# Antibas/eaQHM-analysis-and-synthesis-in-Python

Measured on AMD Instinct MI355X. Metric: analysis_frames_per_sec, higher is better.
Workload: dtype f64; 1 GPU; synth16k_60s_female_maxAdpt5; samples=960000, fs=16000, ls_frames_per_adaptation=63936, adaptations_executed=5, Kmax=59, track_bytes=906240000, parallelism=instants sharded x1 by LS cost; boundary records all-gathered per adaptation

## Files before the change

eaqhm-analysis-and-synthesis-in-python_amd/csrc/eaqhm_ls_tile.hip:

```cpp
#include <type_traits>
#include "eaqhm_ls_common.h"
#include "eaqhm_ls_chol.h"
#include "eaqhm_ls_a0.h"
#include "eaqhm_ls_tilemap.h"
#include "eaqhm_ls_twunits.h"
#include "eaqhm_ls_gather.h"
#include "eaqhm_ls_tilelds.h"

namespace eaqhm {
bool ls_a0tile_fits(const LsArgs& A);
int launch_ls_a0tile(eaqhm_ctx* ctx, LsArgs A);

#define DIAG_OWNER(jb, nt) ((int)TL_DIAG[nt][jb])
#define TL_THREADS 512
#define TL_WAVES 8
#define TL_CW 8
static_assert(TLL_TILE == TL_TILE && TLL_DG_TILE == DG_TILE, "eaqhm_ls_tilelds.h and eaqhm_ls_chol.h disagree");

__device__ inline void fetch_next_header(const LsArgs& A, TlHead* hd, int C, int nbuf, int lane) {
  int* cls = uni(A.cls);
  int item = 0;
  if (lane == 0) item = atomicAdd(cls + 8 + C, 1);
  item = uni(item);
  int f = -1;
  if (item < uni(cls[C])) f = uni(cls[16 + (size_t)C * uni(A.n_frames) + item]);
  if (f >= 0) {
    const int* tab = (lane == 0) ? A.ncol : (lane == 1) ? A.frame_c : (lane == 2) ? A.frame_wl : A.frame_inst;
    if (lane < 4) (&hd->n)[lane] = tab[f];
    const int Kmax = uni(A.Kmax);
    if (lane < TL_NSLOT && lane < Kmax) hd->cols[nbuf][lane] = A.cols[(size_t)f * Kmax + lane];
  }
  if (lane == 0) { hd->f = f; hd->buf = nbuf; hd->cls = C; }
}

__device__ inline void tw_step(d4 (&g)[9], double aR, double aI, double bR, double bI, double nk) {
  const double sA = aR + aI, dB = bI - bR;
  const double naR = nk * aR, naI = nk * aI, nsA = nk * sA;
  const double nbR = nk * bR, nbI = nk * bI, ndB = nk * dB;
  g[0] = __builtin_amdgcn_mfma_f64_16x16x4f64(aR, bR, g[0], 0, 0, 0);
  g[1] = __builtin_amdgcn_mfma_f64_16x16x4f64(aI, bI, g[1], 0, 0, 0);
  g[2] = __builtin_amdgcn_mfma_f64_16x16x4f64(sA, dB, g[2], 0, 0, 0);
  g[3] = __builtin_amdgcn_mfma_f64_16x16x4f64(naR, bR, g[3], 0, 0, 0);
  g[4] = __builtin_amdgcn_mfma_f64_16x16x4f64(naI, bI, g[4], 0, 0, 0);
  g[5] = __builtin_amdgcn_mfma_f64_16x16x4f64(nsA, dB, g[5], 0, 0, 0);
  g[6] = __builtin_amdgcn_mfma_f64_16x16x4f64(naR, nbR, g[6], 0, 0, 0);
  g[7] = __builtin_amdgcn_mfma_f64_16x16x4f64(naI, nbI, g[7], 0, 0, 0);
  g[8] = __builtin_amdgcn_mfma_f64_16x16x4f64(nsA, ndB, g[8], 0, 0, 0);
}

__device__ inline void twu_pair_k3(d4 (&g0)[3], d4 (&g1)[3], d4 (&g2)[3], double aR, double aI, double bR, double bI, double nk) {
  const double sA = aR + aI, dB = bI - bR;
  const double naR = nk * aR, naI = nk * aI, nsA = nk * sA;
  const double nbR = nk * bR, nbI = nk * bI, ndB = nk * dB;
  g0[0] = __builtin_amdgcn_mfma_f64_16x16x4f64(aR, bR, g0[0], 0, 0, 0);
  g0[1] = __builtin_amdgcn_mfma_f64_16x16x4f64(aI, bI, g0[1], 0, 0, 0);
  g0[2] = __builtin_amdgcn_mfma_f64_16x16x4f64(sA, dB, g0[2], 0, 0, 0);
  g1[0] = __builtin_amdgcn_mfma_f64_16x16x4f64(naR, bR, g1[0], 0, 0, 0);
  g1[1] = __builtin_amdgcn_mfma_f64_16x16x4f64(naI, bI, g1[1], 0, 0, 0);
  g1[2] = __builtin_amdgcn_mfma_f64_16x16x4f64(nsA, dB, g1[2], 0, 0, 0);
  g2[0] = __builtin_amdgcn_mfma_f64_16x16x4f64(naR, nbR, g2[0], 0, 0, 0);
  g2[1] = __builtin_amdgcn_mfma_f64_16x16x4f64(naI, nbI, g2[1], 0, 0, 0);
  g2[2] = __builtin_amdgcn_mfma_f64_16x16x4f64(nsA, ndB, g2[2], 0, 0, 0);
}
__device__ inline void twu_pair_2acc(d4 (&g0)[2], d4 (&g1)[2], d4 (&g2)[2], double aR, double aI, double bR, double bI, double nk,
                                     bool k4) {
  const double naR = nk * aR, naI = nk * aI, nbR = nk * bR, nbI = nk * bI;
  g0[0] = __builtin_amdgcn_mfma_f64_16x16x4f64(aR, bR, g0[0], 0, 0, 0);
  g1[0] = __builtin_amdgcn_mfma_f64_16x16x4f64(naR, bR, g1[0], 0, 0, 0);
  g2[0] = __builtin_amdgcn_mfma_f64_16x16x4f64(naR, nbR, g2[0], 0, 0, 0);
  g0[1] = __builtin_amdgcn_mfma_f64_16x16x4f64(aR, bI, g0[1], 0, 0, 0);
  g1[1] = __builtin_amdgcn_mfma_f64_16x16x4f64(naR, bI, g1[1], 0, 0, 0);
  g2[1] = __builtin_amdgcn_mfma_f64_16x16x4f64(naR, nbI, g2[1], 0, 0, 0);
  g0[0] = __builtin_amdgcn_mfma_f64_16x16x4f64(aI, bI, g0[0], 0, 0, 0);
  g1[0] = __builtin_amdgcn_mfma_f64_16x16x4f64(naI, bI, g1[0], 0, 0, 0);
  g2[0] = __builtin_amdgcn_mfma_f64_16x16x4f64(naI, nbI, g2[0], 0, 0, 0);
  if (k4) {
    const double maI = -aI, mnaI = -naI;
    g0[1] = __builtin_amdgcn_mfma_f64_16x16x4f64(maI, bR, g0[1], 0, 0, 0);
    g1[1] = __builtin_amdgcn_mfma_f64_16x16x4f64(mnaI, bR, g1[1], 0, 0, 0);
    g2[1] = __builtin_amdgcn_mfma_f64_16x16x4f64(mnaI, nbR, g2[1], 0, 0, 0);
  }
}

__device__ inline void twu_edge_k4(d4 (&g0)[2], d4 (&g1)[2], double aR, double aI, double bR, double bI, double nk) {
  const double nbR = nk * bR, nbI = nk * bI, maI = -aI;
  g0[0] = __builtin_amdgcn_mfma_f64_16x16x4f64(aR, bR, g0[0], 0, 0, 0);
  g1[0] = __builtin_amdgcn_mfma_f64_16x16x4f64(aR, nbR, g1[0], 0, 0, 0);
  g0[1] = __builtin_amdgcn_mfma_f64_16x16x4f64(aR, bI, g0[1], 0, 0, 0);
  g1[1] = __builtin_amdgcn_mfma_f64_16x16x4f64(aR, nbI, g1[1], 0, 0, 0);
  g0[0] = __builtin_amdgcn_mfma_f64_16x16x4f64(aI, bI, g0[0], 0, 0, 0);
  g1[0] = __builtin_amdgcn_mfma_f64_16x16x4f64(aI, nbI, g1[0], 0, 0, 0);
  g0[1] = __builtin_amdgcn_mfma_f64_16x16x4f64(maI, bR, g0[1], 0, 0, 0);
  g1[1] = __builtin_amdgcn_mfma_f64_16x16x4f64(maI, nbR, g1[1], 0, 0, 0);
}

template <int NS, int TW, int UA = 0, int UB = 0, int TB = 0>
__device__ __attribute__((noinline)) void tile_frame(const LsArgs& A, int TS_, int ldx_max_, double* lds, int f_) {
  constexpr int C = NS == 12 ? 5 : NS == 10 ? 4 : NS == 9 ? 3 : NS == 7 ? 2 : NS == 6 ? 1 : 0;
  static_assert(NS == 12 || NS == 10 || NS == 9 || NS == 7 || NS == 6 || NS == 5, "a register budget per class");
  constexpr bool NEXT_HEAD = NS != 10, REC_ROW = NS == 9;
  const bool pre = uni(f_) < 0;
  const int TS = uni(TS_), ldx_max = uni(ldx_max_);
  const int tid = threadIdx.x, nt_thr = TL_THREADS;
  const int lane = tid & 63;
  const int wave = __builtin_amdgcn_readfirstlane(tid >> 6);
  double* U = uni(lds);
  TlHead* hd = (TlHead*)(U + tl_head_offset());
  const int f = pre ? uni(hd->f) : uni(f_);
  double* Xre = U;
  double* Xim = Xre + (size_t)TS * ldx_max;
  const size_t usize_g = (size_t)2 * TS * ldx_max;
  double* ci = U + usize_g;
  unsigned long long* masks = (unsigned long long*)(ci + (size_t)CI_STRIDE * 52);
  double* PanR = U;
  double* PanI = PanR + TL_NTMAX * TL_TILE;
  double* WtR = PanI + TL_NTMAX * TL_TILE;
  double* WtI = WtR + TL_NTMAX * TL_TILE;
  double* LdR = WtI + TL_NTMAX * TL_TILE;
  double* LdI = LdR + TL_TILE;
  double* Dc = LdI + TL_TILE;
  double* Zc = Dc + DG_TILE;
  double* zv = Zc + DG_TILE;
  double* xv = zv + 2 * 16 * TL_NTMAX;
  double* xs = xv + 32 + TL_HEAD_DOUBLES;
  double* sh = xs + 4 * uni(A.Kcmax);
  double* win = sh + 16;
  double* sig = win + 64 * CI_NCH;
  double* dorig = sig + 64 * CI_NCH;

  const int Npad = ((uni(A.Nmax) + 63) >> 6) << 6;
  double* Qs = uni(A.scratch) + (size_t)blockIdx.x * (size_t)uni((int)A.scratch_stride);
  double* Rs = Qs + (size_t)Npad * uni(A.nmax);
  const bool seeds = uni(hd->seeds) != 0;
  const double w1 = uni(2.0 * M_PI / A.fs);
  const int PE = TS / 2;
  const double* sA = uni(A.s);
  const int lcol = lane & 15, lq = lane >> 4;
  unsigned long long* dbg = uni(A.debug);
  unsigned long long t_prev = 0;

  {
    const int n = pre ? uni(hd->n) : uni(A.ncol[f]);
    const int Kc = 2 * n + 1, Ms = 2 * Kc + 1;
    const int nt = (Ms + 15) >> 4;
    const int c = pre ? uni(hd->c) : uni(A.frame_c[f]), wl = pre ? uni(hd->wl) : uni(A.frame_wl[f]);
    const int inst = pre ? uni(hd->inst) : uni(A.frame_inst[f]);
    const int N = 2 * wl + 1, mid = wl;
    const int T = (Kc + 16) >> 4;
    constexpr int UN = UA + UB;
    constexpr int GA = UA / 3, GB = UB / 3;
    constexpr bool G3 = TW > 0 || UN > 0;
    static_assert(TW == 0 || UN == 0, "whole pairs or units");
    static_assert(UN == 0 || (UA == TWU_UA && UB == TWU_UB), "slot layout of eaqhm_ls_twunits.h");
    static_assert(TB >= 0 && TB < TWU_NTB, "unit table");
    constexpr bool PK = UN > 0 && TWU_PACKED[TB];
    constexpr int EC = 16 * (TWU_TT[TB] - 1);
    const int nb = G3 ? T : nt;
    const int ldx = (nb << 4) + ((nb & 1) ? 0 : 16);
    const int npair = T * (T + 1) / 2;
    const int is = 2 * Kc - 16 * (nt - 1);
    const double f0 = uni(A.f0_stale);
    const int* mycols = pre ? (const int*)hd->cols[uni(hd->buf)] : uni(A.cols) + (size_t)f * uni(A.Kmax);
    const int npairs = mid + 1;

    if (dbg && tid == 0) {
      t_prev = __builtin_amdgcn_s_memtime();
      if (hd->t_last && !uni((int)A.debug_diag)) atomicAdd(dbg + 11, t_prev - hd->t_last);
    }
    double sv[2];
#pragma unroll
    for (int r = 0; r < 2; ++r) {
      const int t = tid + r * nt_thr;
      sv[r] = (t < N) ? sA[(size_t)(c - wl) + t] : 0.0;
    }
    for (int q = tid; q < TS * ldx; q += nt_thr) { Xre[q] = 0.0; Xim[q] = 0.0; }
#pragma unroll
    for (int r = 0; r < 2; ++r) {
      const int t = tid + r * nt_thr;
      if (t < N) { win[t] = window_value(false, t, N); sig[t] = sv[r]; }
    }
    int* gappy = (int*)(masks + (size_t)52 * CI_NCH);
    prepare_slots<CI_STRIDE, TL_WAVES>(A, Qs, Rs, Npad, ci, masks, gappy, mycols, n, N, mid, c, wl, seeds, lane, wave, CI_NCH,
                                       REC_ROW ? hd->fmc : nullptr);
    LS_STAMP(0);

    constexpr int NM3 = (NS <= 7) ? NS : 0;
    d4 accR[NS], accI[NS], acc3[NM3 ? NM3 : 1];
    int tP[NS], tQ[NS];
    bool live[NS];
#pragma unroll
    for (int sl = 0; sl < NS; ++sl) {
      accR[sl] = (d4){0, 0, 0, 0};
      accI[sl] = (d4){0, 0, 0, 0};
      if (sl < NM3) acc3[sl] = (d4){0, 0, 0, 0};
      const int code = TL_MAP[nt][wave][sl];
      live[sl] = code != 0xFF;
      const int P = live[sl] ? (code >> 4) : 0, Q = live[sl] ? (code & 15) : 0;
      tP[sl] = __builtin_amdgcn_readfirstlane(P);
      tQ[sl] = __builtin_amdgcn_readfirstlane(Q);
    }

    constexpr int TWA = TW ? TW : 1;
    const bool split = TW > 0 && NS == 5 && T == 4;
    d4 g[TWA][9];
    int gI[TWA], gJ[TWA], gx[TWA];
    bool glive[TWA];
#pragma unroll
    for (int sl = 0; sl < TWA; ++sl) {
      const int x = (split && sl == 1) ? 8 + (wave >> 1) : wave + 8 * sl;
      glive[sl] = TW && x < npair && !(split && sl == 1 && wave >= 4);
      gx[sl] = __builtin_amdgcn_readfirstlane(x);
      int I = 0, J = 0;
      if (glive[sl]) tile_of(x, I, J);
      gI[sl] = __builtin_amdgcn_readfirstlane(I);
      gJ[sl] = __builtin_amdgcn_readfirstlane(J);
#pragma unroll
      for (int p = 0; p < 9; ++p) g[sl][p] = (d4){0, 0, 0, 0};
    }

    constexpr int UAA = UA > 3 ? UA : 3, UBA = UB > 3 ? UB : 3;
    d4 ga[UAA][3], gb[UBA][2];
    int ucode[UN ? UN : 1];
    if constexpr (UN > 0) {
#pragma unroll
      for (int sl = 0; sl < UN; ++sl) ucode[sl] = __builtin_amdgcn_readfirstlane((int)TWU_MAPS[TB][wave][sl]);
#pragma unroll
      for (int sl = 0; sl < UA; ++sl)
#pragma unroll
        for (int p = 0; p < 3; ++p) ga[sl][p] = (d4){0, 0, 0, 0};
#pragma unroll
      for (int sl = 0; sl < UB; ++sl) gb[sl][0] = gb[sl][1] = (d4){0, 0, 0, 0};
    }

    for (int d0 = 0; d0 < npairs; d0 += PE) {
#pragma clang loop unroll(disable)
      for (int idx = tid; idx < 16 * n; idx += nt_thr) {
        const int el = idx & 15, j = idx >> 4, d = d0 + el;
        const bool act = d <= mid;
        const int u = mid - d - 1, v = mid + d;
        double su = 0, cu = 1, sv, cv;
        double pur = 0, pui = 0, nur = 0, nui = 0, pvr, pvi, nvr, nvi;
        {
          double* cj = ci + j * CI_STRIDE;
          const double* fb = ((const double**)cj)[2];
          const double* ab = ((const double**)cj)[3];
          const int dc = act ? d : mid;
          const double fu1 = fb[mid - dc], fv = fb[mid + dc];
          const double au = ab[(mid - dc - 1 >= 0) ? (mid - dc - 1) : 0], au1 = ab[mid - dc];
          const double av = ab[mid + dc], av1 = ab[(mid + dc + 1 < N) ? (mid + dc + 1) : (N - 1)];
          const double xu = act ? fu1 : 0.0, xv = (act && d >= 1) ? fv : 0.0;
          const double qv = cj[0] + scan16(xv), qu = -(cj[1] + scan16(xu));
          if (el == 15) { cj[0] = qv; cj[1] = -qu; }
          if (!act) continue;
          const double ainv = cj[17], pr = cj[18], pi = cj[19];
          sincos_cw(qu * w1, &su, &cu);
          sincos_cw(qv * w1, &sv, &cv);
          const double eps = 10e-5;
          if (u >= 0) {
            const double ru = (eps + au) * ainv, rv1 = (eps + av1) * ainv;
            pur = ru * cu;                    pui = ru * su;
            nur = rv1 * (cv * pr - sv * pi);  nui = rv1 * (cv * pi + sv * pr);
          }
          const double rv = (eps + av) * ainv, ru1 = (eps + au1) * ainv;
          pvr = rv * cv;                      pvi = rv * sv;
          nvr = ru1 * (cu * pr - su * pi);    nvi = ru1 * (cu * pi + su * pr);
        }
        double* xr = Xre + (2 * el) * ldx;
        double* xi = Xim + (2 * el) * ldx;
        const int cpos = XCOL(n + 1 + j, el), cneg = XCOL(j, el);
        const int spos = XCOL(Kc + n + 1 + j, el), sneg = XCOL(Kc + j, el);
        const double wv = win[v], nv = (double)(v - mid);
        if (u >= 0) {
          const double wu = win[u], nu = (double)(u - mid);
          pur *= wu; pui *= wu; nur *= wu; nui *= wu;
          xr[cpos] = pur;      xi[cpos] = pui;      xr[cneg] = nur;      xi[cneg] = nui;
          if (!G3) { xr[spos] = nu * pur; xi[spos] = nu * pui; xr[sneg] = nu * nur; xi[sneg] = nu * nui; }
          if (PK && n + 1 + j >= EC) { xr[XCOL(n + 9 + j, el)] = nu * pur; xi[XCOL(n + 9 + j, el)] = nu * pui; }
        }
        pvr *= wv; pvi *= wv; nvr *= wv; nvi *= wv;
        xr += ldx; xi += ldx;
        xr[cpos] = pvr;      xi[cpos] = pvi;      xr[cneg] = nvr;      xi[cneg] = nvi;
        if (!G3) { xr[spos] = nv * pvr; xi[spos] = nv * pvi; xr[sneg] = nv * nvr; xi[sneg] = nv * nvi; }
        if (PK && n + 1 + j >= EC) { xr[XCOL(n + 9 + j, el)] = nv * pvr; xi[XCOL(n + 9 + j, el)] = nv * pvi; }
      }
      if ((tid & 15) == 0 && (tid >> 4) < TS) {
        const int row = tid >> 4;
        const int d = d0 + (row >> 1);
        const int t = (row & 1) ? (mid + d) : (mid - d - 1);
        const bool ok = (d <= mid) && (t >= 0);
        const double w = ok ? win[t] : 0.0;
        const double sval = ok ? sig[t] : 0.0;
        const double nn = (double)(t - mid);
        const int el = row >> 1;
        double* xr = Xre + row * ldx;
        double* xi = Xim + row * ldx;
        xr[XCOL(n, el)] = w;               xi[XCOL(n, el)] = 0.0;
        if (!G3) {
          xr[XCOL(Kc + n, el)] = w * nn;   xi[XCOL(Kc + n, el)] = 0.0;
        }
        const int scol = G3 ? Kc : 2 * Kc;
        xr[XCOL(scol, el)] = w * sval;     xi[XCOL(scol, el)] = 0.0;
        if (PK) { xr[XCOL(Kc + 8, el)] = w * sval * nn;  xi[XCOL(Kc + 8, el)] = 0.0; }
      }
      if (d0 + PE > mid) {
        for (int q = tid; q < TS * 16 * nb; q += nt_thr) {
          const int row = q / (16 * nb), col = q - row * (16 * nb);
          const int d = d0 + (row >> 1);
          const int t = (row & 1) ? (mid + d) : (mid - d - 1);
          if (d > mid || t < 0) { Xre[row * ldx + col] = 0.0; Xim[row * ldx + col] = 0.0; }
        }
      }
      LS_STAMP(12);
      __syncthreads();
      LS_STAMP(1);
      const int pcs = (npairs - d0 < PE) ? (npairs - d0) : PE;
      const int ksl = (pcs + 1) >> 1;
      if constexpr (UN > 0) {
        const int plane = TS * ldx_max;
        const int kn = (ksl < 8) ? ksl : 8;
#pragma unroll
        for (int gi = 0; gi < GA + GB; ++gi) {
          const int s0 = (gi < GA) ? 3 * gi : UA + 3 * (gi - GA);
          const int code = ucode[s0];
          if (code == 0xFFFF) continue;
          const int ca = 16 * ((code >> 8) & 15), cb = 16 * ((code >> 4) & 15);
          const bool k4 = (code & 3) == 1;
          int rb = lq * ldx;
          const int sw0 = lcol + (lq >> 1);
          int nk = (lq & 1) ? d0 + (lq >> 1) : -d0 - (lq >> 1) - 1;
          asm volatile("" : "+v"(rb), "+v"(nk));
          if (PK && gi >= GA) {
            if (code & 0x1000) {
              const int q = (gi >= GA) ? 3 * (gi - GA) : 0;
#pragma clang loop unroll(disable)
              for (int ks = 0; ks < kn; ++ks) {
                const int sw = (sw0 + 2 * ks) & 15;
                const double aR = Xre[rb + ca + sw], aI = Xre[rb + ca + sw + plane];
                const double bR = Xre[rb + cb + sw], bI = Xre[rb + cb + sw + plane];
                rb += 4 * ldx;
                twu_edge_k4(gb[q], gb[q + 1], aR, aI, bR, bI, (double)nk);
                nk += (lq & 1) ? 2 : -2;
              }
              continue;
            }
          }
#pragma clang loop unroll(disable)
          for (int ks = 0; ks < kn; ++ks) {
            const int sw = (sw0 + 2 * ks) & 15;
            const double aR = Xre[rb + ca + sw], aI = Xre[rb + ca + sw + plane];
            const double bR = Xre[rb + cb + sw], bI = Xre[rb + cb + sw + plane];
            rb += 4 * ldx;
            if (gi < GA) {
              const int q = (gi < GA) ? 3 * gi : 0;
              twu_pair_k3(ga[q], ga[q + 1], ga[q + 2], aR, aI, bR, bI, (double)nk);
            } else {
              const int q = (gi >= GA) ? 3 * (gi - GA) : 0;
              twu_pair_2acc(gb[q], gb[q + 1], gb[q + 2], aR, aI, bR, bI, (double)nk, k4);
            }
            nk += (lq & 1) ? 2 : -2;
          }
        }
#pragma unroll
        for (int sl = 0; sl < UN; ++sl) {
          if ((sl < UA) ? (sl < 3 * GA) : (sl - UA < 3 * GB)) continue;
          const int code = ucode[sl];
          if (code == 0xFFFF) continue;
          const int ca = 16 * ((code >> 8) & 15), cb = 16 * ((code >> 4) & 15), up = (code >> 2) & 3;
          const bool k4 = (code & 3) == 1;
          int rb = lq * ldx;
          const int sw0 = lcol + (lq >> 1);
          int nk = (lq & 1) ? d0 + (lq >> 1) : -d0 - (lq >> 1) - 1;
          asm volatile("" : "+v"(rb), "+v"(nk));
          auto run = [&](auto pc) {
            constexpr int P = decltype(pc)::value;
#pragma clang loop unroll(disable)
            for (int ks = 0; ks < kn; ++ks) {
              const int sw = (sw0 + 2 * ks) & 15;
              double aR = Xre[rb + ca + sw], aI = Xre[rb + ca + sw + plane];
              double bR = Xre[rb + cb + sw], bI = Xre[rb + cb + sw + plane];
              rb += 4 * ldx;
              if constexpr (P == 1 || P == 2) { aR *= (double)nk; aI *= (double)nk; }
              if constexpr (P >= 2) { bR *= (double)nk; bI *= (double)nk; }
              nk += (lq & 1) ? 2 : -2;
              if (sl < UA) {
                d4 (&g)[3] = ga[sl < UA ? sl : 0];
                g[0] = __builtin_amdgcn_mfma_f64_16x16x4f64(aR, bR, g[0], 0, 0, 0);
                g[1] = __builtin_amdgcn_mfma_f64_16x16x4f64(aI, bI, g[1], 0, 0, 0);
                g[2] = __builtin_amdgcn_mfma_f64_16x16x4f64(aR + aI, bI - bR, g[2], 0, 0, 0);
              } else {
                d4 (&g)[2] = gb[sl >= UA ? sl - UA : 0];
                g[0] = __builtin_amdgcn_mfma_f64_16x16x4f64(aR, bR, g[0], 0, 0, 0);
                g[1] = __builtin_amdgcn_mfma_f64_16x16x4f64(aR, bI, g[1], 0, 0, 0);
                g[0] = __builtin_amdgcn_mfma_f64_16x16x4f64(aI, bI, g[0], 0, 0, 0);
                if (k4) g[1] = __builtin_amdgcn_mfma_f64_16x16x4f64(-aI, bR, g[1], 0, 0, 0);
              }
            }
          };
          if (up == 0) run(std::integral_constant<int, 0>{});
          else if (PK && (code & 0x1000)) run(std::integral_constant<int, PK ? 3 : 1>{});
          else if (up == 1) run(std::integral_constant<int, 1>{});
          else run(std::integral_constant<int, 2>{});
        }
      } else if constexpr (TW > 0) {
#pragma unroll
        for (int sl = 0; sl < TW; ++sl) {
          if (!glive[sl]) continue;
          const int ca = 16 * gI[sl], cb = 16 * gJ[sl];
          int rb = lq * ldx;
          const int sw0 = lcol + (lq >> 1);
          int nk = (lq & 1) ? d0 + (lq >> 1) : -d0 - (lq >> 1) - 1;
          asm volatile("" : "+v"(rb), "+v"(nk));
          const int plane = TS * ldx_max;
          int kn = (ksl < 8) ? ksl : 8;
          int ks = 0;
          if (split && sl == 1) {
            if (wave & 1) { ks = 4; rb += 16 * ldx; nk += (lq & 1) ? 8 : -8; }
            else kn = (kn < 4) ? kn : 4;
          }
#pragma clang loop unroll(disable)
          for (; ks < kn; ++ks) {
            const int sw = (sw0 + 2 * ks) & 15;
            const double aR = Xre[rb + ca + sw], aI = Xre[rb + ca + sw + plane];
            const double bR = Xre[rb + cb + sw], bI = Xre[rb + cb + sw + plane];
            rb += 4 * ldx;
            tw_step(g[sl], aR, aI, bR, bI, (double)nk);
            nk += (lq & 1) ? 2 : -2;
          }
        }
      } else {
#pragma unroll
        for (int sl = 0; sl < NS; ++sl) {
          if (!live[sl]) continue;
          const int ca = 16 * tP[sl], cb = 16 * tQ[sl];
          int rb = lq * ldx;
          const int sw0 = lcol + (lq >> 1);
          asm volatile("" : "+v"(rb));
          const int plane = TS * ldx_max;
          if (ksl < 8) {
#pragma clang loop unroll(disable)
            for (int ks = 0; ks < ksl; ++ks) {
              const int sw = (sw0 + 2 * ks) & 15;
              const double aR = Xre[rb + ca + sw], aI = Xre[rb + ca + sw + plane];
              const double bR = Xre[rb + cb + sw], bI = Xre[rb + cb + sw + plane];
              rb += 4 * ldx;
              if (sl < NM3) {
                accR[sl] = __builtin_amdgcn_mfma_f64_16x16x4f64(aR, bR, accR[sl], 0, 0, 0);
                acc3[sl < NM3 ? sl : 0] = __builtin_amdgcn_mfma_f64_16x16x4f64(aI, bI, acc3[sl < NM3 ? sl : 0], 0, 0, 0);
                accI[sl] = __builtin_amdgcn_mfma_f64_16x16x4f64(aR + aI, bI - bR, accI[sl], 0, 0, 0);
              } else {
                accR[sl] = __builtin_amdgcn_mfma_f64_16x16x4f64(aR, bR, accR[sl], 0, 0, 0);
                accI[sl] = __builtin_amdgcn_mfma_f64_16x16x4f64(aR, bI, accI[sl], 0, 0, 0);
                accR[sl] = __builtin_amdgcn_mfma_f64_16x16x4f64(aI, bI, accR[sl], 0, 0, 0);
                accI[sl] = __builtin_amdgcn_mfma_f64_16x16x4f64(-aI, bR, accI[sl], 0, 0, 0);
              }
            }
            continue;
          }
          double aR, aI, bR, bI;
          {
            const int sw = sw0 & 15;
            aR = Xre[rb + ca + sw]; aI = Xre[rb + ca + sw + plane]; bR = Xre[rb + cb + sw]; bI = Xre[rb + cb + sw + plane];
          }
#pragma unroll
          for (int ks = 0; ks < 8; ++ks) {
            double naR = 0, naI = 0, nbR = 0, nbI = 0;
            if (ks < 7) {
              rb += 4 * ldx;
              const int sw = (sw0 + 2 * (ks + 1)) & 15;
              naR = Xre[rb + ca + sw]; naI = Xre[rb + ca + sw + plane]; nbR = Xre[rb + cb + sw]; nbI = Xre[rb + cb + sw + plane];
            }
            __builtin_amdgcn_sched_barrier(0);
            if (sl < NM3) {
              accR[sl] = __builtin_amdgcn_mfma_f64_16x16x4f64(aR, bR, accR[sl], 0, 0, 0);
              acc3[sl < NM3 ? sl : 0] = __builtin_amdgcn_mfma_f64_16x16x4f64(aI, bI, acc3[sl < NM3 ? sl : 0], 0, 0, 0);
              accI[sl] = __builtin_amdgcn_mfma_f64_16x16x4f64(aR + aI, bI - bR, accI[sl], 0, 0, 0);
            } else {
              accR[sl] = __builtin_amdgcn_mfma_f64_16x16x4f64(aR, bR, accR[sl], 0, 0, 0);
              accI[sl] = __builtin_amdgcn_mfma_f64_16x16x4f64(aR, bI, accI[sl], 0, 0, 0);
              accR[sl] = __builtin_amdgcn_mfma_f64_16x16x4f64(aI, bI, accR[sl], 0, 0, 0);
              accI[sl] = __builtin_amdgcn_mfma_f64_16x16x4f64(-aI, bR, accI[sl], 0, 0, 0);
            }
            aR = naR; aI = naI; bR = nbR; bI = nbI;
          }
        }
      }
      __syncthreads();
      LS_STAMP(2);
    }
    if constexpr (TW == 0 && NM3 > 0) {
#pragma unroll
      for (int sl = 0; sl < NM3; ++sl) {
        const d4 p1 = accR[sl], p2 = acc3[sl];
        accR[sl] = p1 + p2;
        accI[sl] = accI[sl] + (p1 - p2);
      }
    }
    if constexpr (G3) {
      double* Gs = Qs;
      int4* gtab = (int4*)U;
      if (tid < 16 * nt) {
        const GatherEntry e = gather_entry(tid, Kc, npair, T, PK);
        gtab[2 * tid] = make_int4(e.lo, e.hi, e.trow, e.tcol);
        if constexpr (PK) gtab[2 * tid + 1] = make_int4(e.mask, e.val, 0, 0);
      }
      if (tid == TL_THREADS - 1) *(double2*)((char*)Gs + GI_ZCELL) = make_double2(0.0, 0.0);
      if constexpr (UN > 0) {
#pragma unroll
        for (int sl = 0; sl < UN; ++sl) {
          const int code = ucode[sl];
          if (code == 0xFFFF) continue;
          const int I = (code >> 8) & 15, J = (code >> 4) & 15, up = (code >> 2) & 3;
          d4 re, im;
          if (sl < UA) {
            const d4 p1 = ga[sl < UA ? sl : 0][0], p2 = ga[sl < UA ? sl : 0][1];
            re = p1 + p2; im = ga[sl < UA ? sl : 0][2] + (p1 - p2);
          } else {
            re = gb[sl >= UA ? sl - UA : 0][0]; im = gb[sl >= UA ? sl - UA : 0][1];
          }
          double* gt = Gs + (size_t)(up * npair + I * (I + 1) / 2 + J) * 512;
#pragma unroll
          for (int r = 0; r < 4; ++r) {
            const int o = 2 * (16 * (lq + 4 * r) + lcol);
            gt[o] = re[r]; gt[o + 1] = im[r];
          }
        }
      } else
#pragma unroll
      for (int sl = 0; sl < TWA; ++sl) {
        if (!glive[sl]) continue;
        const int x = gx[sl];
        const bool second = split && sl == 1 && (wave & 1);
#pragma unroll
        for (int p = 0; p < 3; ++p) {
          const d4 p1 = g[sl][3 * p], p2 = g[sl][3 * p + 1];
          const d4 re = p1 + p2, im = g[sl][3 * p + 2] + (p1 - p2);
          double* gt = Gs + (size_t)(second ? 3 * npair + 3 * (x - 8) + p : p * npair + x) * 512;
#pragma unroll
          for (int r = 0; r < 4; ++r) {
            const int o = 2 * (16 * (lq + 4 * r) + lcol);
            gt[o] = re[r]; gt[o + 1] = im[r];
          }
        }
      }
      __syncthreads();
      if (split) {
        double2 c1[3], c2[3];
#pragma unroll
        for (int k = 0; k < 3; ++k) {
          const int q = tid + k * TL_THREADS, t = q >> 8, e = 2 * (q & 255);
          c1[k] = *(const double2*)(Gs + (size_t)((t % 3) * npair + 8 + t / 3) * 512 + e);
          c2[k] = *(const double2*)(Gs + (size_t)(3 * npair + t) * 512 + e);
        }
#pragma unroll
        for (int k = 0; k < 3; ++k) {
          const int q = tid + k * TL_THREADS, t = q >> 8, e = 2 * (q & 255);
          *(double2*)(Gs + (size_t)((t % 3) * npair + 8 + t / 3) * 512 + e) = make_double2(c1[k].x + c2[k].x, c1[k].y + c2[k].y);
        }
        __syncthreads();
      }
      if constexpr (UN > 0) {
        constexpr int TT = TWU_TT[TB], HN = (PK ? 3 * (TT - 1) + 1 : 3 * TT) * 136, HF = HN / TL_THREADS, HT = HF + (HN % TL_THREADS ? 1 : 0);
        double ha[HT], hb[HT];
        int hoa[HT], hob[HT];
#pragma unroll
        for (int k = 0; k < HT; ++k) {
          const int q = tid + k * TL_THREADS, qc = (q < HN) ? q : 0;
          const int t = qc / 136, e = qc - 136 * t, r = e / 17, c = e - 17 * r;
          const int i = (c < 16 - r) ? r : 15 - r, j = (c < 16 - r) ? r + c : c - 1;
          const int TD = PK ? TT - 1 : TT, pl = (t < 3 * TD) ? t / TD : 0, I = (t < 3 * TD) ? t - pl * TD : TT - 1;
          const int tile = (pl * npair + I * (I + 1) / 2 + I) * 512;
          hoa[k] = tile + 2 * (16 * i + j) + 1; hob[k] = tile + 2 * (16 * j + i) + 1;
          ha[k] = Gs[hoa[k]]; hb[k] = Gs[hob[k]];
        }
#pragma unroll
        for (int k = 0; k < HT; ++k) {
          if (k < HF || tid + k * TL_THREADS < HN) {
            Gs[hoa[k]] = ha[k] - hb[k];
            Gs[hob[k]] = hb[k] - ha[k];
          }
        }
        __syncthreads();
      }
      typedef const __attribute__((address_space(1))) char* gather_base_t;
      gather_base_t Gb = (gather_base_t)(const char*)Gs;
      unsigned gup[NS];
#pragma unroll
      for (int sl = 0; sl < NS; ++sl) {
        const int cx = live[sl] ? 16 * tQ[sl] + lcol : 16 * nt - 1;
        const int4* rt = gtab + 2 * (16 * tP[sl] + lq);
        int4 c0 = gtab[2 * cx], c1 = make_int4(0, 0, 0, 0), r0[4], r1[4];
        if constexpr (PK) c1 = gtab[2 * cx + 1];
#pragma unroll
        for (int r = 0; r < 4; ++r) {
          r0[r] = rt[8 * r];
          if constexpr (PK) r1[r] = rt[8 * r + 1];
        }
        asm volatile("" : "+v"(c0.x), "+v"(c0.y), "+v"(c0.w));
        if constexpr (PK) asm volatile("" : "+v"(c1.x), "+v"(c1.y));
#pragma unroll
        for (int r = 0; r < 4; ++r) {
          asm volatile("" : "+v"(r0[r].x), "+v"(r0[r].y), "+v"(r0[r].z));
          if constexpr (PK) asm volatile("" : "+v"(r1[r].x), "+v"(r1[r].y));
        }
        unsigned ups = 0;
#pragma unroll
        for (int r = 0; r < 4; ++r) {
          const int dt = r0[r].z - c0.w;
          unsigned off = (unsigned)((dt < 0 ? r0[r].y : r0[r].x) + (dt < 0 ? c0.x : c0.y));
          if constexpr (PK) off += (unsigned)((dt < 0 ? c1.x : r1[r].x) & (dt < 0 ? r1[r].y : c1.y));
          off = off < (unsigned)GI_ZCELL ? off : (unsigned)GI_ZCELL;
          ups = (ups >> 1) | ((unsigned)dt & 0x80000000u);
          typedef double gather_d2 __attribute__((ext_vector_type(2)));
          const gather_d2 v = *(const __attribute__((address_space(1))) gather_d2*)(Gb + off);
          accR[sl][r] = v.x; accI[sl][r] = v.y;
        }
        gup[sl] = ups;
      }
      __builtin_amdgcn_sched_barrier(0);
#pragma unroll
      for (int sl = 0; sl < NS; ++sl) {
#pragma unroll
        for (int r = 0; r < 4; ++r) {
          const double vi = accI[sl][r];
          accI[sl][r] = __hiloint2double(__double2hiint(vi) ^ (int)((gup[sl] << (3 - r)) & 0x80000000u), __double2loint(vi));
        }
      }
      LS_STAMP(uni((int)A.debug_diag) ? 2 : 9);
    }

    {
#pragma unroll
      for (int sl = 0; sl < NS; ++sl) {
        if (!live[sl] || tP[sl] != nt - 1) continue;
#pragma unroll
        for (int r = 0; r < 4; ++r) {
          const int row = lq + 4 * r, col = lcol;
          const bool pad = (row > is) || (tQ[sl] == nt - 1 && col > is);
          if (pad) {
            accR[sl][r] = (tQ[sl] == nt - 1 && row == col) ? 1.0 : 0.0;
            accI[sl][r] = 0.0;
          }
        }
      }
#pragma unroll
      for (int sl = 0; sl < NS; ++sl) {
        if (!live[sl] || tP[sl] != tQ[sl]) continue;
#pragma unroll
        for (int r = 0; r < 4; ++r)
          if (lq + 4 * r == lcol) dorig[16 * tP[sl] + lcol] = accR[sl][r];
      }
      double* post = Dc;
      double* dumpD = Dc + DGP_DOUBLES;
      double* zs = dumpD + 128;
      int* dflag = (int*)(zs + 256);
      if (tid == 0) *dflag = 0;
      __syncthreads();
#define TRAILING_UPDATE(sl)                                                                         \
  {                                                                                                 \
    const double* ar = PanR + tP[sl] * TL_TILE;                                                     \
    const double* ai = PanI + tP[sl] * TL_TILE;                                                     \
    const double* br = PanR + tQ[sl] * TL_TILE;                                                     \
    const double* bi = PanI + tQ[sl] * TL_TILE;                                                     \
       \
       \
    d4 p1 = (d4){0, 0, 0, 0}, p2 = (d4){0, 0, 0, 0};                                                \
    _Pragma("unroll") for (int ks = 0; ks < 4; ++ks) {                                              \
      const int o = (4 * ks + lq) * TL_LD + lcol;                                                   \
      const double aR = ar[o], aI = ai[o], lR = br[o], lI = bi[o];                                  \
      p1 = __builtin_amdgcn_mfma_f64_16x16x4f64(aR, lR, p1, 0, 0, 0);                               \
      p2 = __builtin_amdgcn_mfma_f64_16x16x4f64(aI, lI, p2, 0, 0, 0);                               \
      accI[sl] = __builtin_amdgcn_mfma_f64_16x16x4f64(aR + aI, lI - lR, accI[sl], 0, 0, 0);         \
    }                                                                                               \
    accR[sl] = accR[sl] - (p1 + p2);                                                                \
    accI[sl] = accI[sl] + (p1 - p2);                                                                \
  }
      for (int jb = 0; jb < nt; ++jb) {
        d4 Rt = (d4){0, 0, 0, 0}, It = (d4){0, 0, 0, 0};
        bool mine = false;
#pragma unroll
        for (int sl = 0; sl < NS; ++sl) {
          if (!live[sl] || tP[sl] != jb || tQ[sl] != jb) continue;
          if (jb > 0) TRAILING_UPDATE(sl)
          Rt = accR[sl]; It = accI[sl];
          mine = true;
        }
        if (mine) {
          unsigned long long td0 = 0;
          unsigned long long* tlast = (unsigned long long*)(dflag + 2);
          const bool tdiag = dbg && uni(A.debug_diag);
          if (tdiag) td0 = __builtin_amdgcn_s_memtime();
          diag_D(Rt, It, post, nullptr, dflag, 16 * jb, dumpD, LdR, LdI, jb == nt - 1);
          if (tdiag && lane == 0) {
            const unsigned long long td1 = __builtin_amdgcn_s_memtime();
            atomicAdd(dbg + 9, td1 - td0);
            if (jb > 0) { atomicAdd(dbg + 11, td0 - *tlast); atomicAdd(dbg + 14, 1ull); }
            atomicAdd(dbg + 13, 1ull);
            *tlast = td1;
          }
        }
        LS_STAMP(10);
        if (jb > 0) {
#pragma unroll
          for (int sl = 0; sl < NS; ++sl) {
            if (!live[sl] || tQ[sl] < jb || (tP[sl] == jb && tQ[sl] == jb)) continue;
            TRAILING_UPDATE(sl)
          }
        }
        LS_STAMP(8);
        if (NEXT_HEAD && jb == 0) {
          int pfw = 0;
          while (pfw == DIAG_OWNER(0, nt) || pfw == (int)TL_HELP[nt][0]) ++pfw;
          if (wave == pfw) fetch_next_header(A, hd, C, uni(hd->buf) ^ 1, lane);
        }
        if (!mine && wave == (int)TL_HELP[nt][jb])
          diag_Z(post, dflag, 16 * jb, zs, WtR + jb * TL_TILE, WtI + jb * TL_TILE, dorig + 16 * jb,
                 (jb == nt - 1) ? is : 16, uni(A.fault));
        __syncthreads();
        LS_STAMP(6);
#pragma unroll
        for (int sl = 0; sl < NS; ++sl) {
          if (!live[sl] || tQ[sl] != jb || tP[sl] == jb) continue;
          double* tr = PanR + tP[sl] * TL_TILE;
          double* ti = PanI + tP[sl] * TL_TILE;
#pragma unroll
          for (int r = 0; r < 4; ++r) {
            tr[lcol * TL_LD + lq + 4 * r] = accR[sl][r];
            ti[lcol * TL_LD + lq + 4 * r] = accI[sl][r];
          }
          __builtin_amdgcn_wave_barrier();
          d4 p1 = (d4){0, 0, 0, 0}, p2 = (d4){0, 0, 0, 0}, p3 = (d4){0, 0, 0, 0};
          const double* wr = WtR + jb * TL_TILE;
          const double* wi = WtI + jb * TL_TILE;
#pragma unroll
          for (int ks = 0; ks < 4; ++ks) {
            const int o = (4 * ks + lq) * TL_LD + lcol;
            const double aR = tr[o], aI = ti[o], bR = wr[o], bI = wi[o];
            p1 = __builtin_amdgcn_mfma_f64_16x16x4f64(aR, bR, p1, 0, 0, 0);
            p2 = __builtin_amdgcn_mfma_f64_16x16x4f64(aI, bI, p2, 0, 0, 0);
            p3 = __builtin_amdgcn_mfma_f64_16x16x4f64(aR + aI, bR + bI, p3, 0, 0, 0);
          }
          const d4 xr = p1 - p2, xi = p3 - (p1 + p2);
          accR[sl] = xr; accI[sl] = xi;
          __builtin_amdgcn_wave_barrier();
#pragma unroll
          for (int r = 0; r < 4; ++r) {
            tr[lcol * TL_LD + lq + 4 * r] = xr[r];
            ti[lcol * TL_LD + lq + 4 * r] = xi[r];
          }
        }
        LS_STAMP(7);
        __syncthreads();
      }
#undef TRAILING_UPDATE
      __syncthreads();
      LS_STAMP(3);

#pragma unroll
      for (int sl = 0; sl < NS; ++sl) {
        if (!live[sl] || tP[sl] != nt - 1 || tQ[sl] == nt - 1) continue;
        if (lq == (is & 3)) {
#pragma unroll
          for (int r = 0; r < 4; ++r)
            if (r == (is >> 2)) {
              zv[2 * (16 * tQ[sl] + lcol)] = accR[sl][r];
              zv[2 * (16 * tQ[sl] + lcol) + 1] = -accI[sl][r];
            }
        }
      }
      if (tid < 16) {
        const bool ok = tid < is;
        zv[2 * (16 * (nt - 1) + tid)] = ok ? LdR[is * TL_LD + tid] : 0.0;
        zv[2 * (16 * (nt - 1) + tid) + 1] = ok ? -LdI[is * TL_LD + tid] : 0.0;
      }
      for (int q = tid; q < 4 * Kc; q += nt_thr) xs[q] = 0.0;
      __syncthreads();
      for (int P = nt - 1; P >= 0; --P) {
        if (tid < 256) {
          const int i = tid >> 4, k = tid & 15;
          double xr = 0, xi = 0;
          if (k >= i) {
            const double wr = WtR[P * TL_TILE + i * TL_LD + k], wi = WtI[P * TL_TILE + i * TL_LD + k];
            const double zr = zv[2 * (16 * P + k)], zi = zv[2 * (16 * P + k) + 1];
            xr = wr * zr - wi * zi;
            xi = wr * zi + wi * zr;
          }
          xr = sum16_first(xr); xi = sum16_first(xi);
          if (k == 0) {
            xv[2 * i] = xr; xv[2 * i + 1] = xi;
            const int q = 16 * P + i;
            if (q < 2 * Kc) { xs[2 * q] = xr; xs[2 * q + 1] = xi; }
          }
        }
        __syncthreads();
#pragma unroll
        for (int sl = 0; sl < NS; ++sl) {
          if (!live[sl] || tP[sl] != P || tQ[sl] == P) continue;
          double sr = 0, si = 0;
#pragma unroll
          for (int r = 0; r < 4; ++r) {
            const double xr = xv[2 * (lq + 4 * r)], xi = xv[2 * (lq + 4 * r) + 1];
            const double lr = accR[sl][r], li = accI[sl][r];
            sr += lr * xr + li * xi;
            si += lr * xi - li * xr;
          }
          sr = sum4rows_first(sr); si = sum4rows_first(si);
          if (lq == 0) {
            zv[2 * (16 * tQ[sl] + lcol)] -= sr;
            zv[2 * (16 * tQ[sl] + lcol) + 1] -= si;
          }
        }
        __syncthreads();
      }
      LS_STAMP(4);
    }

    if (REC_ROW && 3 * uni(A.Kmax) + 1 <= TL_NSLOT * CI_NCH)
      write_record<true>(A, xs, sh, mycols, f, n, inst, c, f0, seeds, hd->fmc, (double*)masks);
    else
      write_record(A, xs, sh, mycols, f, n, inst, c, f0, seeds);
    LS_STAMP(5);
    if (dbg && tid == 0) hd->t_last = t_prev;
  }
}

__device__ inline int frame_class(int n) {
  const int nt = (2 * (2 * n + 1) + 1 + 15) >> 4;
  return nt <= 8 ? 0 : nt == 9 ? 1 : nt == 10 ? 2 : nt == 11 ? 3 : nt == 12 ? 4 : nt <= TL_NTMAX ? 5 : LS_BIG_CLASS;
}
extern "C" __global__ void __launch_bounds__(256) eaqhm_ls_classify_kernel(LsArgs A) {
  const int f = blockIdx.x * blockDim.x + threadIdx.x, lane = threadIdx.x & 63;
  int cl = (f < A.n_frames) ? frame_class((A.mode == 0) ? A.frame_K[f] : A.ncol[f]) : -1;
  if (f < A.n_frames) {
    if (!frame_window_ok(A, A.frame_c[f], A.frame_wl[f])) { cl = -1; atomicAdd(A.fault + 2, 1); }
  }
  if (A.mode == 1 && cl >= 0) {
    const long long c = A.frame_c[f], wl = A.frame_wl[f];
    const long long lo = (c - wl - 1 > 0) ? (c - wl - 1) : 0;
    for (long long ch = lo >> 10; ch <= ((c + wl) >> 10); ++ch) A.zflag[ch] = 1;
  }
  for (int c = 0; c < LS_NCLS; ++c) {
    const unsigned long long m = __ballot(cl == c);
    if (m == 0ull) continue;
    int base = 0;
    if (lane == __ffsll((long long)m) - 1) base = atomicAdd(A.cls + c, __popcll(m));
    base = __shfl(base, __ffsll((long long)m) - 1);
    if (cl == c) A.cls[16 + (size_t)c * A.n_frames + base + __popcll(m & ((1ull << lane) - 1ull))] = f;
  }
}

extern "C" __global__ void __launch_bounds__(256) eaqhm_ls_zero_prefix_kernel(const double* __restrict__ fm, long long Lt,
                                                                              long long t_lo, int ch0, int zchunks,
                                                                              const unsigned char* __restrict__ zflag,
                                                                              unsigned short* __restrict__ zloc,
                                                                              int* __restrict__ ztot) {
  __shared__ int wsum[4];
  const int k = blockIdx.y, ch = ch0 + blockIdx.x, tid = threadIdx.x, lane = tid & 63, wave = tid >> 6;
  if (!zflag[ch]) return;
  const long long base = (long long)ch << 10;
  int run = 0;
  for (int p = 0; p < 4; ++p) {
    const long long t = base + 256 * p + tid;
    const bool in = t >= t_lo && t < t_lo + Lt;
// ... 85 lines not shown
```

eaqhm-analysis-and-synthesis-in-python_amd/csrc/eaqhm_ls_tilelds.h:

```cpp
#pragma once
#include <cstddef>

#if defined(__HIPCC__)
#define TLL_HD __host__ __device__
#else
#define TLL_HD
#endif

#define TL_NTMAX 13
#define CI_STRIDE 20
#define CI_NCH 16
#define TL_NSLOT 52
#define TLL_TILE (16 * 17)
#define TLL_DG_TILE (2 * 16 * 17)
#define TL_LDS_LIMIT (159 * 1024)

#define TL_HEAD_GAP 16
struct TlHead {
  double gap[TL_HEAD_GAP];
  double fmc[TL_NSLOT];
  unsigned long long t_last;
  int cls, f, n, c, wl, inst, buf, seeds;
  int cols[2][TL_NSLOT];
  int even[2];
};
static_assert(sizeof(TlHead) % 16 == 0, "TlHead: a multiple of 16 bytes");
#define TL_HEAD_DOUBLES ((sizeof(TlHead) + 7) / 8)

TLL_HD inline size_t tl_usize_c() {
  return (size_t)4 * TL_NTMAX * TLL_TILE + 2 * TLL_TILE + 2 * TLL_DG_TILE + 2 * 16 * TL_NTMAX + 32;
}
TLL_HD inline size_t tl_usize_g(int TS, int ldx_max) {
  return (size_t)2 * TS * ldx_max + (size_t)CI_STRIDE * TL_NSLOT + TL_NSLOT * CI_NCH + 32;
}
TLL_HD inline size_t tl_head_offset() { return tl_usize_c(); }
TLL_HD inline bool tl_layout_ok(int TS, int ldx_max) { return tl_usize_g(TS, ldx_max) <= tl_usize_c() + TL_HEAD_GAP; }
TLL_HD inline size_t tl_lds_doubles(int Kcmax, int TS, int ldx_max) {
  const size_t c = tl_usize_c() + TL_HEAD_DOUBLES, g = tl_usize_g(TS, ldx_max);
  return (c > g ? c : g) + 4 * (size_t)Kcmax + 16 + 2 * 64 * CI_NCH + 16 * TL_NTMAX;
}

inline bool tl_applicable(int Kcmax, int Nmax) {
  return Nmax <= 64 * CI_NCH && tl_layout_ok(32, 16 * TL_NTMAX + 16) && tl_lds_doubles(Kcmax, 32, 16 * TL_NTMAX + 16) * sizeof(double) <= TL_LDS_LIMIT;
}
```

Before: 1.691 million frames/s.

## Exchange twiddle Gram tiles through swizzled LDS rounds with direct per-slot gather

For the whole-pair twiddle path (TW>0), Gram tiles now go into a compact, XOR-swizzled LDS exchange area instead of the padded Qs layout. When T=5 the planes are split across rounds so they fit. The second split-wave contribution is added in place, which removes the separate 3-plane reduction pass. Each slot then gathers its Cholesky tile entries straight from LDS through an index table, applying the transpose sign via bit tricks. The goal is fewer LDS bank conflicts, less LDS traffic and fewer barriers, at the price of extra rounds and barriers for larger T and more complex addressing.

```diff
diff --git a/eaqhm-analysis-and-synthesis-in-python_amd/csrc/eaqhm_ls_tile.hip b/eaqhm-analysis-and-synthesis-in-python_amd/csrc/eaqhm_ls_tile.hip
--- a/eaqhm-analysis-and-synthesis-in-python_amd/csrc/eaqhm_ls_tile.hip
+++ b/eaqhm-analysis-and-synthesis-in-python_amd/csrc/eaqhm_ls_tile.hip
@@ -6,6 +6,7 @@
 #include "eaqhm_ls_twunits.h"
 #include "eaqhm_ls_gather.h"
 #include "eaqhm_ls_tilelds.h"
+#include "eaqhm_ls_tilexch.h"
 
 namespace eaqhm {
 bool ls_a0tile_fits(const LsArgs& A);
@@ -16,6 +17,7 @@
 #define TL_WAVES 8
 #define TL_CW 8
 static_assert(TLL_TILE == TL_TILE && TLL_DG_TILE == DG_TILE, "eaqhm_ls_tilelds.h and eaqhm_ls_chol.h disagree");
+static_assert(TX_DFLAG_BYTE == 8 * (4 * TL_NTMAX * TL_TILE + 2 * TL_TILE + DGP_DOUBLES + 128 + 256), "eaqhm_ls_tilexch.h: where tile_frame puts dflag");
 
 __device__ inline void fetch_next_header(const LsArgs& A, TlHead* hd, int C, int nbuf, int lane) {
   int* cls = uni(A.cls);
@@ -150,6 +152,7 @@
     constexpr int UN = UA + UB;
     constexpr int GA = UA / 3, GB = UB / 3;
     constexpr bool G3 = TW > 0 || UN > 0;
+    constexpr bool LDS_XCH = TW > 0;
     static_assert(TW == 0 || UN == 0, "whole pairs or units");
     static_assert(UN == 0 || (UA == TWU_UA && UB == TWU_UB), "slot layout of eaqhm_ls_twunits.h");
     static_assert(TB >= 0 && TB < TWU_NTB, "unit table");
@@ -495,7 +498,121 @@
         accI[sl] = accI[sl] + (p1 - p2);
       }
     }
-    if constexpr (G3) {
+    if constexpr (LDS_XCH) {
+      constexpr int PPR = NS == 5 ? 3 : 2, NR = NS == 5 ? 1 : 2;
+      static_assert(PPR == tx_planes_per_round(NS == 5 ? 4 : 5) && NR == tx_rounds(NS == 5 ? 4 : 5), "rounds of eaqhm_ls_tilexch.h");
+      typedef __attribute__((address_space(3))) char* xch_base_t;
+      typedef int xch_i4 __attribute__((ext_vector_type(4)));
+      typedef double xch_d2 __attribute__((ext_vector_type(2)));
+      typedef __attribute__((address_space(3))) xch_d2* xch_cell_t;
+      xch_base_t Xb = (xch_base_t)(char*)U;
+      const unsigned tabB = (unsigned)tx_table_byte(uni(A.Kcmax)), zcB = (unsigned)tx_zcell_byte(uni(A.Kcmax));
+      const __attribute__((address_space(3))) xch_i4* gtab = (const __attribute__((address_space(3))) xch_i4*)(Xb + tabB);
+      if (tid < 16 * nt) {
+        const GatherEntry e = gather_entry(tid, Kc, npair, T, false);
+        *(__attribute__((address_space(3))) xch_i4*)(Xb + tabB + 32 * tid) = (xch_i4){e.lo, e.hi, e.trow, e.tcol};
+      }
+      if (tid == TL_THREADS - 1) *(xch_cell_t)(Xb + zcB) = (xch_d2){0.0, 0.0};
+      const unsigned span = (unsigned)(PPR * TX_TILE_BYTES * npair);
+      static_assert(NR == 1 || (NR == 2 && PPR == 2), "a round after the first holds G_2 alone");
+      unsigned gup[NS];
+#pragma unroll
+      for (int rd = 0; rd < NR; ++rd) {
+#pragma unroll
+        for (int sl = 0; sl < TWA; ++sl) {
+          if (!glive[sl]) continue;
+          const bool second = split && sl == 1 && (wave & 1);
+          if (second) continue;
+#pragma unroll
+          for (int p = 0; p < 3; ++p) {
+            if (p / PPR != rd) continue;
+            const d4 p1 = g[sl][3 * p], p2 = g[sl][3 * p + 1];
+            const d4 re = p1 + p2, im = g[sl][3 * p + 2] + (p1 - p2);
+            const unsigned tb = (unsigned)(TX_TILE_BYTES * ((p % PPR) * npair + gx[sl]));
+#pragma unroll
+            for (int r = 0; r < 4; ++r)
+              *(xch_cell_t)(Xb + tb + tx_swizzle((unsigned)(256 * (lq + 4 * r) + 16 * lcol))) = (xch_d2){re[r], im[r]};
+          }
+        }
+        __syncthreads();
+        if (NS == 5 && split) {
+          if (glive[TWA - 1] && (wave & 1)) {
+#pragma unroll
+            for (int p = 0; p < 3; ++p) {
+              const d4 p1 = g[TWA - 1][3 * p], p2 = g[TWA - 1][3 * p + 1];
+              const d4 re = p1 + p2, im = g[TWA - 1][3 * p + 2] + (p1 - p2);
+              const unsigned tb = (unsigned)(TX_TILE_BYTES * (p * npair + gx[TWA - 1]));
+              xch_d2 c1[4];
+#pragma unroll
+              for (int r = 0; r < 4; ++r) c1[r] = *(xch_cell_t)(Xb + tb + tx_swizzle((unsigned)(256 * (lq + 4 * r) + 16 * lcol)));
+#pragma unroll
+              for (int r = 0; r < 4; ++r)
+                *(xch_cell_t)(Xb + tb + tx_swizzle((unsigned)(256 * (lq + 4 * r) + 16 * lcol))) = (xch_d2){c1[r].x + re[r], c1[r].y + im[r]};
+            }
+          }
+          __syncthreads();
+        }
+#pragma unroll
+        for (int sl = 0; sl < NS; ++sl) {
+          if (rd > 0) {
+            const int r0 = 16 * tP[sl], c0 = 16 * tQ[sl];
+            if (!(r0 + 15 >= Kc && r0 < 2 * Kc && c0 + 15 >= Kc && c0 < 2 * Kc)) continue;
+          }
+          unsigned off[4];
+          {
+            const int cx = live[sl] ? 16 * tQ[sl] + lcol : 16 * nt - 1;
+            const __attribute__((address_space(3))) xch_i4* rt = gtab + 2 * (16 * tP[sl] + lq);
+            xch_i4 c0 = gtab[2 * cx], r0[4];
+#pragma unroll
+            for (int r = 0; r < 4; ++r) r0[r] = rt[8 * r];
+            asm volatile("" : "+v"(c0.x), "+v"(c0.y), "+v"(c0.w));
+#pragma unroll
+            for (int r = 0; r < 4; ++r) asm volatile("" : "+v"(r0[r].x), "+v"(r0[r].y), "+v"(r0[r].z));
+            unsigned ups = 0;
+#pragma unroll
+            for (int r = 0; r < 4; ++r) {
+              const int dt = r0[r].z - c0.w;
+              const unsigned o = (unsigned)((dt < 0 ? r0[r].y : r0[r].x) + (dt < 0 ? c0.x : c0.y));
+              off[r] = o < (unsigned)GI_ZCELL ? o : (unsigned)GI_ZCELL;
+              ups = (ups >> 1) | ((unsigned)dt & 0x80000000u);
+            }
+            if (rd == 0) gup[sl] = ups;
+          }
+          if (rd == 0) {
+#pragma unroll
+            for (int r = 0; r < 4; ++r) {
+              const xch_d2 v = *(xch_cell_t)(Xb + (off[r] < span ? tx_swizzle(off[r]) : zcB));
+              accR[sl][r] = v.x; accI[sl][r] = v.y;
+            }
+          } else {
+            bool in[4];
+            xch_d2 v[4];
+#pragma unroll
+            for (int r = 0; r < 4; ++r) {
+              off[r] -= (unsigned)rd * span;
+              in[r] = off[r] < span;
+              v[r] = *(xch_cell_t)(Xb + (in[r] ? tx_swizzle(off[r]) : zcB));
+            }
+#pragma unroll
+            for (int r = 0; r < 4; ++r) {
+              accR[sl][r] = in[r] ? v[r].x : accR[sl][r];
+              accI[sl][r] = in[r] ? v[r].y : accI[sl][r];
+            }
+          }
+        }
+        if (rd + 1 < NR) __syncthreads();
+      }
+#pragma unroll
+      for (int sl = 0; sl < NS; ++sl) {
+#pragma unroll
+        for (int r = 0; r < 4; ++r) {
+          const double vi = accI[sl][r];
+          accI[sl][r] = __hiloint2double(__double2hiint(vi) ^ (int)((gup[sl] << (3 - r)) & 0x80000000u), __double2loint(vi));
+        }
+      }
+      LS_STAMP(uni((int)A.debug_diag) ? 2 : 9);
+    }
+    if constexpr (G3 && !LDS_XCH) {
       double* Gs = Qs;
       int4* gtab = (int4*)U;
       if (tid < 16 * nt) {
@@ -524,40 +641,8 @@
             gt[o] = re[r]; gt[o + 1] = im[r];
           }
         }
-      } else
-#pragma unroll
-      for (int sl = 0; sl < TWA; ++sl) {
-        if (!glive[sl]) continue;
-        const int x = gx[sl];
-        const bool second = split && sl == 1 && (wave & 1);
-#pragma unroll
-        for (int p = 0; p < 3; ++p) {
-          const d4 p1 = g[sl][3 * p], p2 = g[sl][3 * p + 1];
-          const d4 re = p1 + p2, im = g[sl][3 * p + 2] + (p1 - p2);
-          double* gt = Gs + (size_t)(second ? 3 * npair + 3 * (x - 8) + p : p * npair + x) * 512;
-#pragma unroll
-          for (int r = 0; r < 4; ++r) {
-            const int o = 2 * (16 * (lq + 4 * r) + lcol);
-            gt[o] = re[r]; gt[o + 1] = im[r];
-          }
-        }
       }
       __syncthreads();
-      if (split) {
-        double2 c1[3], c2[3];
-#pragma unroll
-        for (int k = 0; k < 3; ++k) {
-          const int q = tid + k * TL_THREADS, t = q >> 8, e = 2 * (q & 255);
-          c1[k] = *(const double2*)(Gs + (size_t)((t % 3) * npair + 8 + t / 3) * 512 + e);
-          c2[k] = *(const double2*)(Gs + (size_t)(3 * npair + t) * 512 + e);
-        }
-#pragma unroll
-        for (int k = 0; k < 3; ++k) {
-          const int q = tid + k * TL_THREADS, t = q >> 8, e = 2 * (q & 255);
-          *(double2*)(Gs + (size_t)((t % 3) * npair + 8 + t / 3) * 512 + e) = make_double2(c1[k].x + c2[k].x, c1[k].y + c2[k].y);
-        }
-        __syncthreads();
-      }
       if constexpr (UN > 0) {
         constexpr int TT = TWU_TT[TB], HN = (PK ? 3 * (TT - 1) + 1 : 3 * TT) * 136, HF = HN / TL_THREADS, HT = HF + (HN % TL_THREADS ? 1 : 0);
         double ha[HT], hb[HT];
diff --git a/eaqhm-analysis-and-synthesis-in-python_amd/csrc/eaqhm_ls_tilelds.h b/eaqhm-analysis-and-synthesis-in-python_amd/csrc/eaqhm_ls_tilelds.h
--- a/eaqhm-analysis-and-synthesis-in-python_amd/csrc/eaqhm_ls_tilelds.h
+++ b/eaqhm-analysis-and-synthesis-in-python_amd/csrc/eaqhm_ls_tilelds.h
@@ -27,7 +27,7 @@
 static_assert(sizeof(TlHead) % 16 == 0, "TlHead: a multiple of 16 bytes");
 #define TL_HEAD_DOUBLES ((sizeof(TlHead) + 7) / 8)
 
-TLL_HD inline size_t tl_usize_c() {
+TLL_HD constexpr inline size_t tl_usize_c() {
   return (size_t)4 * TL_NTMAX * TLL_TILE + 2 * TLL_TILE + 2 * TLL_DG_TILE + 2 * 16 * TL_NTMAX + 32;
 }
 TLL_HD inline size_t tl_usize_g(int TS, int ldx_max) {
diff --git a/eaqhm-analysis-and-synthesis-in-python_amd/csrc/eaqhm_ls_tilexch.h b/eaqhm-analysis-and-synthesis-in-python_amd/csrc/eaqhm_ls_tilexch.h
--- /dev/null
+++ b/eaqhm-analysis-and-synthesis-in-python_amd/csrc/eaqhm_ls_tilexch.h
@@ -0,0 +1,44 @@
+#pragma once
+#include "eaqhm_ls_gather.h"
+#include "eaqhm_ls_tilelds.h"
+
+#define TX_TILE_BYTES 4096
+#define TX_TILES 30
+#define TX_BYTES (TX_TILES * TX_TILE_BYTES)
+#define TX_DFLAG_BYTE (8 * (4 * TL_NTMAX * TLL_TILE + 2 * TLL_TILE + 512 + 128 + 256))
+#define TX_DFLAG_CELL 16
+#define TX_TABLE_BYTES (32 * 16 * TL_NTMAX)
+#define TX_MAX_CONFLICT 2
+#define TX_MAX_CONFLICT_MIXED 4
+
+GI_HD constexpr inline int tx_planes_per_round(int T) { return T <= 4 ? 3 : T == 5 ? 2 : T == 6 ? 1 : 0; }
+GI_HD constexpr inline int tx_rounds(int T) { return T <= 4 ? 1 : T == 5 ? 2 : 3; }
+GI_HD constexpr inline int tx_npair(int T) { return T * (T + 1) / 2; }
+
+static_assert(3 * tx_npair(4) * TX_TILE_BYTES <= TX_BYTES, "T = 4: one round");
+static_assert(tx_planes_per_round(5) * tx_npair(5) * TX_TILE_BYTES <= TX_BYTES, "T = 5: two planes in a round");
+static_assert(tx_planes_per_round(6) * tx_npair(6) * TX_TILE_BYTES <= TX_BYTES, "T = 6: one plane in a round");
+static_assert(TX_BYTES <= TX_DFLAG_BYTE, "dflag's cell lies behind the exchange area");
+static_assert(TX_DFLAG_BYTE + TX_DFLAG_CELL <= 8 * tl_usize_c(), "dflag's cell lies in region U");
+static_assert(TX_TABLE_BYTES <= 8 * 64 * CI_NCH, "the index table fits the analysis window's area");
+
+GI_HD inline size_t tx_table_byte(int Kcmax) { return 8 * (tl_usize_c() + TL_HEAD_DOUBLES + 4 * (size_t)Kcmax + 16); }
+GI_HD inline size_t tx_zcell_byte(int Kcmax) { return tx_table_byte(Kcmax) + 8 * 64 * CI_NCH; }
+
+GI_HD inline unsigned tx_swizzle(unsigned off) { return off ^ (((off >> 8) & 15u) << 4); }
+
+GI_HD inline unsigned tx_entry_addr(int q, int pair, int i, int j, int T) {
+  const int slot = (q % tx_planes_per_round(T)) * tx_npair(T) + pair;
+  return tx_swizzle((unsigned)(TX_TILE_BYTES * slot + 256 * i + 16 * j));
+}
+GI_HD inline int tx_round_of_plane(int q, int T) { return q / tx_planes_per_round(T); }
+
+GI_HD inline int tx_round_of(unsigned off, int T) {
+  return off >= (unsigned)GI_ZCELL ? 0 : (int)(off / (unsigned)(TX_TILE_BYTES * tx_npair(T))) / tx_planes_per_round(T);
+}
+GI_HD inline unsigned tx_read_addr(unsigned off, int T, int rd, unsigned zcell, bool* take) {
+  const unsigned span = (unsigned)(tx_planes_per_round(T) * TX_TILE_BYTES * tx_npair(T)), rel = off - (unsigned)rd * span;
+  const bool in = rel < span && off < (unsigned)GI_ZCELL;
+  *take = in || (rd == 0 && off >= (unsigned)GI_ZCELL);
+  return in ? tx_swizzle(rel) : zcell;
+}
```

Measured after the change: 1.711 million frames/s (median of 6 runs). 1.2% higher.
